# chaeyeongyun/VQ_SEG

Hardware: AMD Instinct MI355X
Metric: train images/sec @512x512 vqreptunet1x1 K=512 (higher is better)
Workload: dtype bf16; 1 GPU; CPS training iteration (2 x vqreptunet1x1, ResNet-50 encoder, K=[0,0,512,512,512], v1 recipe: 6 forwards + 4 backwards + 2 Adam steps) on 512x512x3 images -- BASELINE configs[2] (the metric's configuration): vqreptunet1x1 512x512, K = 512; labelled_per_gpu=32, unlabelled_per_gpu=32, parallelism=dp1, collectives=none (one process), conv_dtype=bf16

## Files before the change

### vq_seg_amd/csrc/conv_device.h

```cpp
#pragma once
#include <hip/hip_runtime.h>

#include "conv_kernels.h"

namespace vqseg {

typedef float f32x16 __attribute__((ext_vector_type(16)));
typedef float f32x4 __attribute__((ext_vector_type(4)));
typedef float f32x2 __attribute__((ext_vector_type(2)));
typedef __bf16 bf16x8 __attribute__((ext_vector_type(8)));
typedef __bf16 bf16x4 __attribute__((ext_vector_type(4)));
typedef unsigned int u32x4 __attribute__((ext_vector_type(4)));
typedef unsigned int u32x2 __attribute__((ext_vector_type(2)));

__device__ __forceinline__ unsigned int pack2(float a, float b) {
    const __bf16 x = (__bf16)a, y = (__bf16)b;
    return (unsigned int)__builtin_bit_cast(unsigned short, x) | ((unsigned int)__builtin_bit_cast(unsigned short, y) << 16);
}
__device__ __forceinline__ void unpack8(const u32x4 a, float (&v)[8]) {
#pragma unroll
    for (int e = 0; e < 4; ++e) {
        v[2 * e] = __builtin_bit_cast(float, a[e] << 16);
        v[2 * e + 1] = __builtin_bit_cast(float, a[e] & 0xFFFF0000u);
    }
// ... 9 lines not shown
__device__ __forceinline__ void split_row(long m, int hw, long M, int& n, int& rem) {
    if (M <= 0x7fffffffL) {
        const unsigned int um = (unsigned int)m;
        n = (int)(um / (unsigned int)hw);
        rem = (int)(um - (unsigned int)n * (unsigned int)hw);
    } else {
        n = (int)(m / hw);
        rem = (int)(m - (long)n * hw);
    }
}

__device__ __forceinline__ int reflect_idx(int i, int n) {
    if (i < 0) i = -i;
    if (i >= n) i = 2 * n - 2 - i;
    return i;
}

struct ASource {
    const char* src;
    int csrc, cbase;
};
__device__ __forceinline__ ASource a_source(const ConvArgs& p, int ci) {
    const bool second = ci >= p.C1;
    ASource a;
    a.src = reinterpret_cast<const char*>(second ? p.x2 : p.x);
    a.csrc = second ? (p.Cin - p.C1) : p.C1;
    a.cbase = second ? (ci - p.C1) : ci;
    if (p.s3_in) {
        const int cs2 = 2 * (second ? p.s3_cs2 : p.s3_cs1);
        a.csrc = cs2;
        if (a.cbase >= cs2) a.cbase -= cs2;
    }
    return a;
}

__device__ __forceinline__ long out_row(const ConvArgs& p, long m) {
    if (!p.omap) return m;
    const unsigned hw = (unsigned)(p.Ho * p.Wo), um = (unsigned)m;
    const unsigned n = um / hw, rem = um - n * hw;
    const unsigned oh = rem / (unsigned)p.Wo, ow = rem - oh * (unsigned)p.Wo;
    if (p.omap_fold) {
        const int i = 2 * (int)oh + p.omap_ph, j = 2 * (int)ow + p.omap_pw, H = p.omap_h, W = p.omap_w;
        const long body = (long)p.N * H * W;
        if (i >= 1 && j >= 1 && i <= H && j <= W) return ((long)n * H + i - 1) * W + j - 1;
        if (p.omap_fold == 1) {
            const int rl = W + 1 + H;
            if (i == 0 && j <= W) return body + (long)n * rl + j;
            if (j == 0 && i <= H) return body + (long)n * rl + W + i;
            return body + (long)p.N * rl;
        }
        return body;
    }
    return ((long)n * p.omap_h + 2 * oh + p.omap_ph) * p.omap_w + 2 * ow + p.omap_pw;
}

#ifndef GLDS_ABL
#define GLDS_ABL 0
#endif
struct LinearRows {
    long m0;
    __device__ __forceinline__ long operator()(int row) const { return m0 + row; }
};

template <int TBM, int BN, bool PRECISE, int MT, int NTT, int NT, int NTHR, typename RowMap = LinearRows, bool S3 = false, bool FAST = true>
__device__ __forceinline__ void conv_epilogue(f32x16 (&acc)[MT][NTT], const ConvArgs& p, char* smem, long M, long m0, int co0,
                                              int wm, int wn, int r, int h, int tid, RowMap row_to_m = LinearRows{-1}) {
// ... 256 lines not shown
```

### vq_seg_amd/csrc/conv_host.hip

```cpp
#include <hip/hip_runtime.h>
#include <stdlib.h>

#include "conv_internal.h"
#include "options.h"

namespace vqseg {

ConvOptions g_conv_opt;

static const Option CONV_OPTIONS[] = {
    {"conv3x3_patch_min_workgroups", &g_conv_opt.patch_min_wgs},
    {"conv_wgrad1x1_narrow", &g_conv_opt.wgrad1x1_narrow},
    {"stem_fused", &g_conv_opt.stem_fused, OPT_FLAG},
    {"conv_wgrad_round_pct", &g_conv_opt.wgrad_round_pct, OPT_RANGE_KEEP, 10, 400},
    {"conv_wgrad_xcd", &g_conv_opt.wgrad_xcd},
    {"conv_dgrad_s2_merge", &g_conv_opt.dgrad_s2_merge, OPT_FLAG},
    {"conv_wgrad3x3_fill", &g_conv_opt.wgrad3x3_fill},
    {"conv_wgrad3x3_stride2", &g_conv_opt.wgrad3x3_s2},
    {"conv_short_k_small_tile", &g_conv_opt.short_k_small},
    {"conv_short_k_single_buffer", &g_conv_opt.short_k_single},
    {"conv3x3_patch_unroll", &g_conv_opt.patch_unroll},
    {"conv_linear_prologue", &g_conv_opt.glds_lin, OPT_FLAG},
    {"conv_xcd_pair", &g_conv_opt.glds_pair},
    {"conv3x3_patch_xcd_pair", &g_conv_opt.patch_pair, OPT_FLAG},
    {"conv3x3_patch_chunk_stage", &g_conv_opt.patch_chunk_stage, OPT_FLAG},
    {"conv3x3_patch_tile512", &g_conv_opt.patch_tile512},
    {"conv3x3_patch_tile512_launches", &g_conv_opt.patch_tile512_launches},
    {"conv3x3_patch_tile512_min_workgroups", &g_conv_opt.patch_tile512_min_wgs},
    {"conv3x3_patch_wide_tile_s3", &g_conv_opt.patch_wide_s3, OPT_FLAG},
    {"conv3x3_patch_wide_tile", &g_conv_opt.patch_wide, OPT_FLAG},
    {"conv_last_variant", &g_conv_opt.last_variant},
};

int conv_set_option(const char* key, int value) { return apply_option(CONV_OPTIONS, key, value); }

struct ConvProfile {
    bool enabled = false;
    int capacity = 0, count = 0;
    hipEvent_t* ev = nullptr;
    double* flops = nullptr;
    int* kind = nullptr;
    int* shape = nullptr;
};
static ConvProfile g_cprof;

hipError_t conv_profile_begin(int capacity) {
    conv_profile_release();
    g_cprof.ev = (hipEvent_t*)malloc(sizeof(hipEvent_t) * 2 * (size_t)capacity);
    g_cprof.flops = (double*)malloc(sizeof(double) * (size_t)capacity);
    g_cprof.kind = (int*)malloc(sizeof(int) * (size_t)capacity);
    g_cprof.shape = (int*)malloc(sizeof(int) * 4 * (size_t)capacity);
    if (!g_cprof.ev || !g_cprof.flops || !g_cprof.kind || !g_cprof.shape) return hipErrorOutOfMemory;
    for (int i = 0; i < 2 * capacity; ++i) {
        hipError_t rc = hipEventCreate(&g_cprof.ev[i]);
        if (rc != hipSuccess) return rc;
    }
    g_cprof.capacity = capacity;
    g_cprof.count = 0;
    g_cprof.enabled = true;
    return hipSuccess;
}

void conv_profile_release() {
// ... 46 lines not shown
```

### vq_seg_amd/csrc/conv_igemm.hip

```cpp
#include <hip/hip_runtime.h>
#include <stdint.h>

#include "conv_device.h"
#include "conv_internal.h"

namespace vqseg {

constexpr int BM = 128;

template <int BN, bool PRECISE, int BK, bool S3 = false>
__global__ __launch_bounds__(256) void conv_igemm_kernel(const ConvArgs p) {
    constexpr int BKP = BK + 8;
    constexpr int NT = BN / 64;
    constexpr int WN = (BN >= 64) ? 2 : 1;
    constexpr int WM = 4 / WN;
    constexpr int MT = BM / (WM * 32);
    constexpr int NTT = (BN >= 64) ? NT : 1;
    constexpr int A_EPC = PRECISE ? 4 : 8;
    constexpr int A_CPR = BK / A_EPC;
    constexpr int A_RPP = 256 / A_CPR;
    constexpr int A_PASSES = BM / A_RPP;
    constexpr int B_CPR = BK / 8;
    constexpr int B_CHUNKS = BN * B_CPR * (PRECISE ? 2 : 1);
    constexpr int B_PER_THREAD = (B_CHUNKS + 255) / 256;
// ... 160 lines not shown
            }
#pragma unroll
            for (int a = 0; a < MT; ++a)
#pragma unroll
                for (int b = 0; b < NTT; ++b) {
                    if (PRECISE) {
                        acc[a][b] = __builtin_amdgcn_mfma_f32_32x32x16_bf16(a_lo[a], b_hi[b], acc[a][b], 0, 0, 0);
                        acc[a][b] = __builtin_amdgcn_mfma_f32_32x32x16_bf16(a_hi[a], b_lo[b], acc[a][b], 0, 0, 0);
                    }
                    acc[a][b] = __builtin_amdgcn_mfma_f32_32x32x16_bf16(a_hi[a], b_hi[b], acc[a][b], 0, 0, 0);
                }
        }
    };

    load_stage(0, a_r0, b_r0);
    if (n_stage > 1) load_stage(1, a_r1, b_r1);
    store_stage(0, a_r0, b_r0);
    __syncthreads();
    for (int s = 0; s < n_stage; s += 2) {
        if (s + 2 < n_stage) load_stage(s + 2, a_r0, b_r0);
        compute(0);
        if (s + 1 < n_stage) store_stage(1, a_r1, b_r1);
        __syncthreads();
        if (s + 1 >= n_stage) break;
        if (s + 3 < n_stage) load_stage(s + 3, a_r1, b_r1);
        compute(1);
        if (s + 2 < n_stage) store_stage(0, a_r0, b_r0);
        __syncthreads();
    }

    conv_epilogue<BM, BN, PRECISE, MT, NTT, NT, 256, LinearRows, S3, false>(acc, p, smem, M, m0, co0, wm, wn, r, h, tid);
}

template <int TBM, int BN, int NW, int NBUF, int MINW = 1, bool S3 = false, bool LIN = false, bool CLS = false>
__global__ __launch_bounds__(NW * 64, MINW) void conv_igemm_glds_kernel(const ConvArgs pk) {
    ConvArgs pc;
    long cls_tile0 = 0;
    if constexpr (CLS) {
        pc = pk;
        int c = 0;
        while (c + 1 < pk.n_cls && blockIdx.x >= pk.cls[c].tile_end) ++c;
        cls_tile0 = c ? pk.cls[c - 1].tile_end : 0;
        const ConvArgs::Cls& k = pk.cls[c];
        pc.KH = k.KH, pc.KW = k.KW, pc.pad = k.pad, pc.pad_w = k.pad_w, pc.Ho = k.Ho, pc.Wo = k.Wo;
        pc.omap_ph = k.ph, pc.omap_pw = k.pw;
        pc.w_hi = pk.w_hi + k.w_off;
    }
    const ConvArgs& p = CLS ? pc : pk;
    constexpr int BK = 64;
    constexpr int WN = (BN >= 256) ? 4 : (BN >= 64 ? 2 : 1);
    constexpr int WM = NW / WN;
    constexpr int MT = TBM / (WM * 32);
    constexpr int NT = (BN >= 64) ? BN / (WN * 32) : 1;
    constexpr int NTT = NT;
    constexpr int STAGE_BYTES = (TBM + BN) * BK * 2;
    constexpr int A_INSTR = TBM / 8 / NW;
    constexpr int B_ROWS_PER_WAVE = BN / NW;
    constexpr int B_INSTR = (B_ROWS_PER_WAVE + 7) / 8;

    extern __shared__ __attribute__((aligned(16))) char smem[];
    const int tid = threadIdx.x;
    const int lane = tid & 63;
    const int wave = __builtin_amdgcn_readfirstlane(tid >> 6);
    const int wm = wave / WN, wn = wave % WN;
    const int r = lane & 31, h = lane >> 5;

    const long M = (long)p.N * p.Ho * p.Wo;
    long m_tile = blockIdx.x - cls_tile0;
// ... 14 lines not shown
#pragma unroll
    for (int i = 0; i < A_INSTR; ++i) {
        const int trow = 8 * (A_INSTR * wave + i) + (lane >> 3);
        long m = m0 + trow;
        a_ok[i] = m < M;
        a_chunk[i] = slot ^ ((trow >> 1) & 7);
        if constexpr (LIN) {
            a_pix[i] = a_ok[i] ? m : -1;
            a_n[i] = a_oh[i] = a_ow[i] = 0;
        } else {
            if (!a_ok[i]) m = M - 1;
            int n, rem;
            split_row(m, p.Ho * p.Wo, M, n, rem);
            a_n[i] = n;
            a_oh[i] = rem / p.Wo;
            a_ow[i] = rem - a_oh[i] * p.Wo;
            if (p.ring) {
                const int q = rem, wp = p.ring_w, hp = p.ring_h;
                if (q < wp) a_oh[i] = 0, a_ow[i] = q;
                else if (q < 2 * wp) a_oh[i] = hp - 1, a_ow[i] = q - wp;
                else if (q < 2 * wp + hp - 2) a_oh[i] = 1 + (q - 2 * wp), a_ow[i] = 0;
                else a_oh[i] = 1 + (q - 2 * wp - (hp - 2)), a_ow[i] = wp - 1;
            }
        }
    }
    unsigned w_off[B_INSTR];
#pragma unroll
    for (int i = 0; i < B_INSTR; ++i) {
        const int b_row = B_ROWS_PER_WAVE * wave + 8 * i + (lane >> 3);
        const int co = co0 + b_row;
        const bool ok = co < p.Cout && b_row < B_ROWS_PER_WAVE * (wave + 1);
        w_off[i] = ok ? ((unsigned)co * (unsigned)(p.KH * p.KW * ((p.Cin + 31) / 32 * 32)) + (unsigned)((slot ^ ((b_row >> 1) & 7)) << 3)) * 2u
                      : ~0u;
    }

    f32x16 acc[MT][NTT];
#pragma unroll
    for (int a = 0; a < MT; ++a)
#pragma unroll
        for (int b = 0; b < NTT; ++b)
#pragma unroll
            for (int i = 0; i < 16; ++i) acc[a][b][i] = 0.0f;

    const int n_taps = p.KH * p.KW;
    const int cin_p = (p.Cin + 31) / 32 * 32;
    const int chunks_per_tap = p.Cin / BK;
    const int n_stage = n_taps * chunks_per_tap;
    const char* zero = reinterpret_cast<const char*>(g_zero_page);

    int cur_tap = LIN ? 0 : -1;
    auto set_tap = [&](int tap) {
        const int kh = tap / p.KW, kw = tap - kh * p.KW;
#pragma unroll
        for (int i = 0; i < A_INSTR; ++i) {
            int ih = a_oh[i] * p.stride - p.pad + kh;
            int iw = a_ow[i] * p.stride - p.pad_w + kw;
            bool ok = a_ok[i];
            if (p.reflect) {
                ih = reflect_idx(ih, p.H * p.up);
                iw = reflect_idx(iw, p.W * p.up);
            }
            if (p.up == 2) {
                ok = ok && ih >= 0 && iw >= 0 && !((ih | iw) & 1);
                ih >>= 1;
                iw >>= 1;
            }
            ok = ok && ih >= 0 && ih < p.H && iw >= 0 && iw < p.W;
            a_pix[i] = ok ? ((long)a_n[i] * p.H + ih) * p.W + iw : -1;
        }
        cur_tap = tap;
    };

    auto stage = [&](int s, int buf) {
        char* As = smem + buf * STAGE_BYTES;
        char* Bs = As + TBM * BK * 2;
        const int tap = s / chunks_per_tap;
        const int ci0 = (s - tap * chunks_per_tap) * BK;
        if (tap != cur_tap) set_tap(tap);
        const ASource as = a_source(p, ci0);
        const char* src = as.src;
        const int csrc = as.csrc, cbase = as.cbase;
#pragma unroll
        for (int i = 0; i < A_INSTR; ++i) {
            const long off = a_pix[i] * csrc + cbase + a_chunk[i] * 8;
            if (!(GLDS_ABL & 8)) glds16(a_pix[i] >= 0 ? src + off * 2 : zero, As + (A_INSTR * wave + i) * 1024);
        }
        const char* wbase = reinterpret_cast<const char*>(p.w_hi) + ((long)tap * cin_p + ci0) * 2;
#pragma unroll
        for (int i = 0; i < B_INSTR; ++i)
            glds16(w_off[i] != ~0u ? wbase + w_off[i] : zero, Bs + (B_ROWS_PER_WAVE * wave + 8 * i) * 128);
    };

    auto compute = [&](int buf) {
        const char* As = smem + buf * STAGE_BYTES;
        const char* Bs = As + TBM * BK * 2;
#pragma unroll MT * NTT >= 8 ? 1 : 4
        for (int kk = 0; kk < BK / 16; ++kk) {
            bf16x8 af[MT], bfr[NTT];
#pragma unroll
            for (int a = 0; a < MT; ++a) {
                const int row = (wm * MT + a) * 32 + r;
                const int sl = (kk * 2 + h) ^ ((row >> 1) & 7);
                af[a] = *reinterpret_cast<const bf16x8*>(As + row * 128 + sl * 16);
            }
#pragma unroll
            for (int b = 0; b < NTT; ++b) {
                const int row = (BN >= 64 ? (wn * NT + b) * 32 : 0) + r;
                const int sl = (kk * 2 + h) ^ ((row >> 1) & 7);
                bfr[b] = *reinterpret_cast<const bf16x8*>(Bs + row * 128 + sl * 16);
            }
#pragma unroll
            for (int a = 0; a < MT; ++a)
#pragma unroll
                for (int b = 0; b < NTT; ++b)
                    acc[a][b] = __builtin_amdgcn_mfma_f32_32x32x16_bf16(af[a], bfr[b], acc[a][b], 0, 0, 0);
        }
    };

    constexpr int G = A_INSTR + B_INSTR;
    auto wait_in_flight = [&](int stages) {
        if (stages >= 2 && NBUF >= 4) __builtin_amdgcn_s_waitcnt(((2 * G) & 0xF) | (((2 * G) >> 4) << 14) | 0x0F70);
        else if (stages >= 1 && NBUF >= 3) __builtin_amdgcn_s_waitcnt((G & 0xF) | ((G >> 4) << 14) | 0x0F70);
        else __builtin_amdgcn_s_waitcnt(0x0F70);
    };
    if constexpr (NBUF == 1) {
        for (int s = 0; s < n_stage; ++s) {
            stage(s, 0);
            __builtin_amdgcn_s_waitcnt(0x0F70);
// ... 114 lines not shown
    const __bf16* blrow = Bl + (wn * 32 + r) * KPW + h * 8;
#pragma unroll
    for (int kk = 0; kk < NK; ++kk) {
        const int g8 = 2 * kk + h;
        int kh = (g8 * 11) >> 5;
        const int j0 = 8 * (g8 - 3 * kh);
        if (kh > 6) kh = 6;
        const __bf16* src = strip + kh * ROW + j0;
        const bf16x8 b = *reinterpret_cast<const bf16x8*>(brow + kk * 16);
        bf16x8 bl;
        if constexpr (S3) bl = *reinterpret_cast<const bf16x8*>(blrow + kk * 16);
#pragma unroll
        for (int a = 0; a < 2; ++a) {
            const unsigned* sp = reinterpret_cast<const unsigned*>(src + 6 * ((wm * 2 + a) * 32 + r));
            const bf16x8 ah = __builtin_bit_cast(bf16x8, u32x4{sp[0], sp[1], sp[2], sp[3]});
            acc[a][0] = __builtin_amdgcn_mfma_f32_32x32x16_bf16(ah, b, acc[a][0], 0, 0, 0);
            if constexpr (S3) {
                const unsigned* sl = sp + PLANE / 2;
                const bf16x8 al = __builtin_bit_cast(bf16x8, u32x4{sl[0], sl[1], sl[2], sl[3]});
                acc[a][0] = __builtin_amdgcn_mfma_f32_32x32x16_bf16(al, b, acc[a][0], 0, 0, 0);
                acc[a][0] = __builtin_amdgcn_mfma_f32_32x32x16_bf16(ah, bl, acc[a][0], 0, 0, 0);
            }
        }
    }
    __syncthreads();
#if STEM_ABL & 2
    if (acc[0][0][0] != 12345.678f) return;
#endif
    conv_epilogue<TP, 64, false, 2, 1, 1, 256, LinearRows, S3, true>(acc, p, smem, M, m0, 0, wm, wn, r, h, tid);
}

template <int TBM, int BN, int NW, int NBUF, int MINW, bool LIN>
static void launch_glds_lin(const ConvArgs& a, hipStream_t st) {
    const int n_stage = a.KH * a.KW * (a.Cin / 64);
    size_t lds = (size_t)(TBM + BN) * 64 * 2 * (n_stage < NBUF ? n_stage : NBUF);
    const size_t out_tile = (size_t)TBM * (BN + 8) * 2 * (a.out_s3 ? 2 : 1);
    if (out_tile > lds) lds = out_tile;
    const long M = (long)a.N * a.Ho * a.Wo;
    const long m_tiles = (M + TBM - 1) / TBM;
    const int chunks = (a.Cout + BN - 1) / BN;
    if (chunks > 1 && chunks <= g_conv_opt.glds_pair && m_tiles < (1L << 30)) {
        ConvArgs b = a;
        b.pair_chunks = chunks;
        b.pair_tiles = (int)m_tiles;
        const dim3 grid1((unsigned)((m_tiles + 7) / 8 * 8 * chunks));
        g_conv_opt.last_variant = conv_variant_glds(TBM, BN, NW, NBUF, MINW, a.out_s3, LIN, false, true);
        if (a.out_s3) hipLaunchKernelGGL((conv_igemm_glds_kernel<TBM, BN, NW, NBUF, MINW, true, LIN>), grid1, dim3(NW * 64), lds, st, b);
        else hipLaunchKernelGGL((conv_igemm_glds_kernel<TBM, BN, NW, NBUF, MINW, false, LIN>), grid1, dim3(NW * 64), lds, st, b);
        return;
    }
    dim3 grid((unsigned)m_tiles, (unsigned)chunks);
    g_conv_opt.last_variant = conv_variant_glds(TBM, BN, NW, NBUF, MINW, a.out_s3, LIN, false, false);
    if (a.out_s3) hipLaunchKernelGGL((conv_igemm_glds_kernel<TBM, BN, NW, NBUF, MINW, true, LIN>), grid, dim3(NW * 64), lds, st, a);
    else hipLaunchKernelGGL((conv_igemm_glds_kernel<TBM, BN, NW, NBUF, MINW, false, LIN>), grid, dim3(NW * 64), lds, st, a);
}

template <int TBM, int BN, int NW, int NBUF, int MINW = 1>
static void launch_glds_t(const ConvArgs& a, hipStream_t st) {
    const bool lin = g_conv_opt.glds_lin && a.KH == 1 && a.KW == 1 && a.stride == 1 && a.pad == 0 && a.pad_w == 0 && a.up == 1 && !a.omap &&
                     a.Ho == a.H && a.Wo == a.W;
    if (lin) launch_glds_lin<TBM, BN, NW, NBUF, MINW, true>(a, st);
    else launch_glds_lin<TBM, BN, NW, NBUF, MINW, false>(a, st);
}

template <int BN, bool PRECISE, int BK>
static void launch_t(const ConvArgs& a, hipStream_t st) {
    constexpr int BKP = BK + 8;
    size_t lds = (size_t)(BM + BN) * BKP * 2 * (PRECISE ? 2 : 1) * 2;
    const size_t out_tile = (size_t)BM * (BN + (PRECISE ? 4 : 8)) * (PRECISE ? 4 : 2);
    if (out_tile > lds) lds = out_tile;
    const long M = (long)a.N * a.Ho * a.Wo;
    dim3 grid((unsigned)((M + BM - 1) / BM), (unsigned)((a.Cout + BN - 1) / BN));
    g_conv_opt.last_variant = conv_variant_igemm(BN, PRECISE, BK, !PRECISE && a.out_s3);
    if constexpr (!PRECISE) {
        if (a.out_s3) {
            const size_t s3_tile = (size_t)BM * (BN + 8) * 2 * 2;
            if (s3_tile > lds) lds = s3_tile;
            hipLaunchKernelGGL((conv_igemm_kernel<BN, PRECISE, BK, true>), grid, dim3(256), lds, st, a);
            return;
        }
    }
    hipLaunchKernelGGL((conv_igemm_kernel<BN, PRECISE, BK>), grid, dim3(256), lds, st, a);
}

#ifndef SHORTK_MINW
#define SHORTK_MINW 4
// ... 228 lines not shown
```

### vq_seg_amd/csrc/conv_internal.h

```cpp
#pragma once
#include "conv_kernels.h"

namespace vqseg {

struct ConvOptions {
    int glds_pair = 8;
    int glds_lin = 1;
    int patch_min_wgs = 128;
    int patch_pair = 0;
    int patch_chunk_stage = 1;
    int patch_wide_s3 = 1;
    int patch_wide = 1;
    int short_k_small = 1;
    int short_k_single = 8;
    int patch_tile512 = 2;
    int patch_tile512_min_wgs = 512;
    int patch_tile512_launches = 0;
    int patch_unroll = 1;
    int wgrad1x1_narrow = 1;
    int wgrad_round_pct = 100;
    int wgrad_xcd = 1;
    int wgrad3x3_fill = 1;
    int wgrad3x3_s2 = 1;
    int stem_fused = 1;
    int dgrad_s2_merge = 1;
    int last_variant = 0;
};
extern ConvOptions g_conv_opt;

enum ConvFamily { CONV_FAM_GLDS = 1, CONV_FAM_IGEMM = 2, CONV_FAM_PATCH = 3, CONV_FAM_WGRAD3X3 = 4, CONV_FAM_WGRAD1X1 = 5, CONV_FAM_WGRAD_TAP = 6 };
constexpr int conv_variant_id(int family, int d5, int d4, int d3, int d2, int d1, int flags) {
    return family << 24 | d5 << 20 | d4 << 16 | d3 << 12 | d2 << 8 | d1 << 4 | flags;
}
constexpr int conv_variant_glds(int tbm, int bn, int nw, int nbuf, int minw, bool s3, bool lin, bool cls, bool pair) {
    return conv_variant_id(CONV_FAM_GLDS, tbm / 128, bn / 32, nw, nbuf, minw, s3 * 8 + lin * 4 + cls * 2 + pair);
}
constexpr int conv_variant_igemm(int bn, bool precise, int bk, bool s3) { return conv_variant_id(CONV_FAM_IGEMM, 0, bn / 32, 0, bk / 32, precise, s3 * 8); }
constexpr int conv_variant_patch(int bn, int nbw, bool unroll, int ck, bool s3, int tbm, bool pair) {
    return conv_variant_id(CONV_FAM_PATCH, tbm / 256, bn / 32, nbw, ck / 32, unroll, s3 * 8 + pair);
}
constexpr int conv_variant_wgrad3x3(int cot, int cit, int stride, bool xcd) { return conv_variant_id(CONV_FAM_WGRAD3X3, 0, cot, cit, stride, 0, xcd); }
constexpr int conv_variant_wgrad1x1(int cot, int cit, bool xcd) { return conv_variant_id(CONV_FAM_WGRAD1X1, 0, cot, cit, 0, 0, xcd); }
constexpr int conv_variant_wgrad_tap(int tm, int tn, bool precise) { return conv_variant_id(CONV_FAM_WGRAD_TAP, 0, tm, tn, 0, precise, 0); }

class ConvProfileScope {
public:
    ConvProfileScope(hipStream_t st, double flops, int kind, int shape0, int shape1, int shape2, int shape3);
    ~ConvProfileScope();
    ConvProfileScope(const ConvProfileScope&) = delete;
    ConvProfileScope& operator=(const ConvProfileScope&) = delete;

private:
    hipStream_t st_;
    int slot_;
};

bool launch_conv3x3_patch(const ConvArgs& a, bool k64, hipStream_t st);

}
```

### vq_seg_amd/csrc/conv_patch.hip

```cpp
#include <hip/hip_runtime.h>
#include <stdint.h>

#include "conv_device.h"
#include "conv_internal.h"

namespace vqseg {

#ifndef PATCH_ABL
#define PATCH_ABL 0
#endif
#ifndef CONV_SETPRIO
#define CONV_SETPRIO 0
#endif

template <int BN, int NBW, bool UNROLL_TAPS, int CK = 64, bool S3 = false, int TBM = 256>
__global__ __launch_bounds__(512) void conv3x3_patch_kernel(const ConvArgs p) {
    constexpr int NW = 8;
    static_assert(TBM == 256 || (TBM == 512 && CK == 32), "512-pixel tiles stage 32-channel chunks (two patch buffers must fit the LDS)");
    constexpr int PATCH_PX = TBM == 256 ? 344 : 616;
    constexpr int NT = BN >= 128 ? 2 : 1;
    constexpr int WN = BN / (32 * NT), WM = NW / WN;
    constexpr int MT = TBM / (WM * 32);
    constexpr int ROWB = CK * 2;
    constexpr int RPI = 1024 / ROWB;
    constexpr int KS = CK / 16;
    constexpr int PI = (PATCH_PX + RPI * NW - 1) / (RPI * NW);
    constexpr int PATCH_BYTES = PI * NW * 1024;
    constexpr int W_ROWS = (BN * ROWB >= NW * 1024) ? BN : NW * 1024 / ROWB;
    constexpr int W_BYTES = W_ROWS * ROWB;
    constexpr int WI = W_BYTES / 1024 / NW;
    static_assert(W_BYTES % (1024 * NW) == 0 && (CK == 64 || CK == 32), "weight tile must split evenly over the waves");
    constexpr bool CHUNK_STAGE = NBW == 0;
    constexpr int WT_BYTES = CHUNK_STAGE ? BN * ROWB : W_BYTES;
    constexpr int WCI = 9 * BN * ROWB / 1024, WCW = (WCI + NW - 1) / NW;
    static_assert(!CHUNK_STAGE || (BN * ROWB) % 1024 == 0, "a tap's weight tile must be whole DMA instructions");
    auto swz = [](int row) { return CK == 64 ? ((row >> 1) & 7) : ((row >> 2) & 3); };

    extern __shared__ __attribute__((aligned(16))) char smem[];
    char* const patch0 = smem;
    char* const wring = smem + ((CHUNK_STAGE && p.Cin / CK == 1) ? 1 : 2) * PATCH_BYTES;
    const int tid = threadIdx.x, lane = tid & 63;
    const int wave = __builtin_amdgcn_readfirstlane(tid >> 6);
    const int wm = wave / WN, wn = wave % WN;
    const int r = lane & 31, h = lane >> 5;

    const int tw_shift = (p.W & 31) == 0 ? 5 : 4;
    const int TW = 1 << tw_shift, TH = TBM >> tw_shift, PW = TW + 2, PH = TH + 2;
    const int tiles_x = p.W >> tw_shift, tiles_y = p.H / TH;
    int tile_id = blockIdx.x, co_chunk = blockIdx.y;
    if (p.pair_chunks > 0) {
        const unsigned group = 8u * (unsigned)p.pair_chunks, within = blockIdx.x % group;
        tile_id = (int)(blockIdx.x / group) * 8 + (int)(within & 7u);
        co_chunk = (int)(within >> 3);
        if (tile_id >= p.pair_tiles) return;
    }
    int t = tile_id;
    const int txi = t % tiles_x;
    t /= tiles_x;
    const int tyi = t % tiles_y;
    const int n = t / tiles_y;
    const int oh0 = tyi * TH, ow0 = txi * TW;
    const int co0 = co_chunk * BN;

    const int slot = lane & (ROWB / 16 - 1), lrow = lane / (ROWB / 16);
    unsigned w_off[WI];
#pragma unroll
    for (int i = 0; i < WI; ++i) {
        const int row = RPI * (wave * WI + i) + lrow;
        int co = co0 + row;
        co = co < p.Cout ? co : p.Cout - 1;
        w_off[i] = ((unsigned)co * (unsigned)(9 * ((p.Cin + 31) / 32 * 32)) + (unsigned)((slot ^ swz(row)) << 3)) * 2u;
    }
    int a_pp[MT];
#pragma unroll
    for (int a = 0; a < MT; ++a) {
        const int row = (wm * MT + a) * 32 + r;
        a_pp[a] = (row >> tw_shift) * PW + (row & (TW - 1));
    }

    f32x16 acc[MT][NT];
#pragma unroll
    for (int a = 0; a < MT; ++a)
#pragma unroll
        for (int b = 0; b < NT; ++b)
#pragma unroll
            for (int i = 0; i < 16; ++i) acc[a][b][i] = 0.0f;

    const int cin_p = (p.Cin + 31) / 32 * 32;
    const int n_chunks = p.Cin / CK;
    const int n_stage = n_chunks * 9;
    const char* zero = reinterpret_cast<const char*>(g_zero_page);

    auto issue_patch = [&](int chunk, int i) {
        const int pp = RPI * (wave + NW * i) + lrow;
        const int pr = pp / PW, pc = pp - pr * PW;
        int ih = oh0 - 1 + pr, iw = ow0 - 1 + pc;
        bool ok = pr < PH;
        if (p.reflect && ok) {
            ih = reflect_idx(ih, p.H);
            iw = reflect_idx(iw, p.W);
        }
        ok = ok && ih >= 0 && ih < p.H && iw >= 0 && iw < p.W;
        const long pix = ((long)n * p.H + ih) * p.W + iw;
        const int ci0 = chunk * CK;
        const ASource as = a_source(p, ci0);
        const char* src = as.src;
        const int csrc = as.csrc, cbase = as.cbase;
        const long off = pix * csrc + cbase + ((slot ^ swz(pp)) << 3);
        glds16(ok ? src + off * 2 : zero, patch0 + (chunk & 1) * PATCH_BYTES + (wave + NW * i) * 1024);
    };
    auto issue_weights = [&](int chunk, int tap, int wslot) {
        char* Bs = wring + wslot * W_BYTES;
        const char* sbase = reinterpret_cast<const char*>(p.w_hi) + ((long)tap * cin_p + chunk * CK) * 2;
#pragma unroll
        for (int i = 0; i < WI; ++i) glds16(sbase + w_off[i], Bs + (wave * WI + i) * 1024);
    };
    auto compute = [&](int chunk, int tapoff, const char* Bs) {
        const char* Ps = patch0 + (chunk & 1) * PATCH_BYTES;
#pragma unroll
        for (int kk = 0; kk < KS; ++kk) {
            bf16x8 af[MT], bfr[NT];
#pragma unroll
            for (int a = 0; a < MT; ++a) {
                const int pp = a_pp[a] + tapoff;
                af[a] = *reinterpret_cast<const bf16x8*>(Ps + pp * ROWB + (((kk * 2 + h) ^ swz(pp)) << 4));
            }
#pragma unroll
            for (int b = 0; b < NT; ++b) {
                const int row = (wn * NT + b) * 32 + r;
                bfr[b] = *reinterpret_cast<const bf16x8*>(Bs + row * ROWB + (((kk * 2 + h) ^ swz(row)) << 4));
            }
#if CONV_SETPRIO
            __builtin_amdgcn_s_setprio(1);
#endif
#pragma unroll
            for (int a = 0; a < MT; ++a)
#pragma unroll
                for (int b = 0; b < NT; ++b)
                    acc[a][b] = __builtin_amdgcn_mfma_f32_32x32x16_bf16(af[a], bfr[b], acc[a][b], 0, 0, 0);
#if CONV_SETPRIO
            __builtin_amdgcn_s_setprio(0);
#endif
        }
    };

    if constexpr (CHUNK_STAGE) {
        auto issue_chunk = [&](int chunk) {
#pragma unroll
            for (int i = 0; i < PI; ++i) issue_patch(chunk, i);
            char* wb = wring + (chunk & 1) * (9 * WT_BYTES);
#pragma unroll
            for (int i = 0; i < WCW; ++i) {
                const int j = wave * WCW + i;
                if (j < WCI) {
                    const int tap = j / (BN * ROWB / 1024), rg = j % (BN * ROWB / 1024);
                    const int row = RPI * rg + lrow;
                    int co = co0 + row;
                    co = co < p.Cout ? co : p.Cout - 1;
                    const unsigned short* wp = p.w_hi + (long)co * (9L * cin_p) + (long)tap * cin_p + chunk * CK + ((slot ^ swz(row)) << 3);
                    glds16(reinterpret_cast<const char*>(wp), wb + j * 1024);
                }
            }
        };
        issue_chunk(0);
        for (int chunk = 0; chunk < n_chunks; ++chunk) {
            __builtin_amdgcn_s_waitcnt(0x0F70);
            stage_barrier();
            if (chunk + 1 < n_chunks) issue_chunk(chunk + 1);
            const char* wb = wring + (chunk & 1) * (9 * WT_BYTES);
#pragma unroll
            for (int tap = 0; tap < 9; ++tap) compute(chunk, (tap / 3) * PW + tap % 3, wb + tap * WT_BYTES);
        }
        __syncthreads();
        const long M = (long)p.N * p.H * p.W;
        const TileRows rows{((long)n * p.H + oh0) * p.W + ow0, tw_shift, p.W};
        conv_epilogue<TBM, BN, false, MT, NT, NT, NW * 64, TileRows, S3>(acc, p, smem, M, (long)tile_id * TBM, co0, wm, wn, r, h, tid, rows);
        return;
    }
#pragma unroll
    for (int i = 0; i < PI; ++i) issue_patch(0, i);
#pragma unroll
    for (int s = 0; s < NBW - 1; ++s)
        if (s < n_stage) issue_weights(s / 9, s % 9, s);

    int wslot = 0;
    for (int chunk = 0; chunk < n_chunks; ++chunk) {
        const bool more = chunk + 1 < n_chunks;
#pragma unroll UNROLL_TAPS ? 9 : 1
        for (int tap = 0; tap < 9; ++tap) {
            const int s = chunk * 9 + tap;
            int young = 0;
#pragma unroll
// ... 19 lines not shown
                    const int c2 = tap + NBW - 1 >= 9 ? chunk + 1 : chunk, t2 = tap + NBW - 1 >= 9 ? tap + NBW - 1 - 9 : tap + NBW - 1;
                    int ws2 = wslot + NBW - 1;
                    if (ws2 >= NBW) ws2 -= NBW;
                    issue_weights(c2, t2, ws2);
                }
            };
            if (NBW < 4) issue_next();
            compute(chunk, (tap / 3) * PW + tap % 3, wring + wslot * W_BYTES);
            if (NBW >= 4) issue_next();
            wslot = wslot == NBW - 1 ? 0 : wslot + 1;
        }
    }
    __syncthreads();
    const long M = (long)p.N * p.H * p.W;
    const TileRows rows{((long)n * p.H + oh0) * p.W + ow0, tw_shift, p.W};
    conv_epilogue<TBM, BN, false, MT, NT, NT, NW * 64, TileRows, S3>(acc, p, smem, M, (long)tile_id * TBM, co0, wm, wn, r, h, tid, rows);
}

static bool conv3x3_patch_ok(const ConvArgs& a) {
    if (a.omap || a.pad_w != a.pad) return false;
    if (a.KH != 3 || a.KW != 3 || a.stride != 1 || a.pad != 1 || a.up != 1 || a.Ho != a.H || a.Wo != a.W) return false;
    const int ck = a.Cin % 64 == 0 && (a.C1 == a.Cin || a.C1 % 64 == 0) ? 64 : 32;
    if (a.Cin % ck || (a.C1 != a.Cin && a.C1 % ck) || (a.Cout % 128 && a.Cout != 64 && a.Cout != 32)) return false;
    const int tw = (a.W % 32 == 0) ? 32 : 16, th = 256 / tw;
    if (a.W % tw || a.H % th) return false;
    const int bn = a.Cout % 128 == 0 ? 128 : a.Cout;
    return (long)a.N * (a.H / th) * (a.W / tw) * (a.Cout / bn) >= g_conv_opt.patch_min_wgs;
}

template <int BN, int NBW, bool UNROLL_TAPS, int CK = 64, int TBM = 256>
static void launch_patch_t(const ConvArgs& a, hipStream_t st) {
    constexpr int ROWB = CK * 2, RPI = 1024 / ROWB, PI = ((TBM == 256 ? 344 : 616) + RPI * 8 - 1) / (RPI * 8);
    constexpr int W_ROWS = (BN * ROWB >= 8 * 1024) ? BN : 8 * 1024 / ROWB;
    size_t lds = 2 * (size_t)PI * 8 * 1024 + (size_t)NBW * W_ROWS * ROWB;
    if (NBW == 0) {
        const int nb = a.Cin / CK > 1 ? 2 : 1;
        lds = (size_t)nb * ((size_t)PI * 8 * 1024 + 9 * (size_t)BN * ROWB);
    }
    size_t out_tile = (size_t)TBM * (BN + 8) * 2 * (a.out_s3 ? 2 : 1);
    if (a.out_s3 && out_tile > 160u * 1024u) out_tile = (size_t)TBM * (BN / 2 + 8) * 4;
    if (out_tile > lds) lds = out_tile;
    const int tw = (a.W % 32 == 0) ? 32 : 16, th = TBM / tw;
    const long tiles = (long)a.N * (a.H / th) * (a.W / tw);
    const int chunks = a.Cout / BN;
    if (g_conv_opt.patch_pair && chunks > 1) {
        ConvArgs b = a;
        b.pair_chunks = chunks;
        b.pair_tiles = (int)tiles;
        const dim3 grid1((unsigned)((tiles + 7) / 8 * 8 * chunks));
        g_conv_opt.last_variant = conv_variant_patch(BN, NBW, UNROLL_TAPS, CK, a.out_s3, TBM, true);
        if (a.out_s3) hipLaunchKernelGGL((conv3x3_patch_kernel<BN, NBW, UNROLL_TAPS, CK, true, TBM>), grid1, dim3(512), lds, st, b);
        else hipLaunchKernelGGL((conv3x3_patch_kernel<BN, NBW, UNROLL_TAPS, CK, false, TBM>), grid1, dim3(512), lds, st, b);
        return;
    }
    dim3 grid((unsigned)tiles, (unsigned)chunks);
    g_conv_opt.last_variant = conv_variant_patch(BN, NBW, UNROLL_TAPS, CK, a.out_s3, TBM, false);
    if (a.out_s3) hipLaunchKernelGGL((conv3x3_patch_kernel<BN, NBW, UNROLL_TAPS, CK, true, TBM>), grid, dim3(512), lds, st, a);
    else hipLaunchKernelGGL((conv3x3_patch_kernel<BN, NBW, UNROLL_TAPS, CK, false, TBM>), grid, dim3(512), lds, st, a);
}

static bool conv3x3_tile512_ok(const ConvArgs& a, int bn) {
    if (a.Cin % 32 || (a.C1 != a.Cin && a.C1 % 32)) return false;
    const int tw = (a.W % 32 == 0) ? 32 : 16, th = 512 / tw;
    if (a.W % tw || a.H % th) return false;
    if (a.out_s3 && (size_t)512 * (bn + 8) * 2 * 2 > 160 * 1024) return false;
    return (long)a.N * (a.H / th) * (a.W / tw) * (a.Cout / bn) >= g_conv_opt.patch_tile512_min_wgs;
}

bool launch_conv3x3_patch(const ConvArgs& a, bool k64, hipStream_t st) {
    if (!conv3x3_patch_ok(a)) return false;
    if ((g_conv_opt.patch_tile512 & 2) && (a.Cout == 32 || (a.Cout == 64 && a.Cin >= 64)) && conv3x3_tile512_ok(a, a.Cout)) {
        ++g_conv_opt.patch_tile512_launches;
        if (a.Cout == 64) launch_patch_t<64, 0, true, 32, 512>(a, st);
        else launch_patch_t<32, 0, true, 32, 512>(a, st);
    } else if (!k64) {
        if (g_conv_opt.patch_chunk_stage && a.Cout == 64) launch_patch_t<64, 0, true, 32>(a, st);
        else if (g_conv_opt.patch_chunk_stage && a.Cout == 32) launch_patch_t<32, 0, true, 32>(a, st);
        else if (g_conv_opt.patch_chunk_stage && a.Cin == 32) launch_patch_t<128, 0, true, 32>(a, st);
        else if (a.Cout == 64) launch_patch_t<64, 3, true, 32>(a, st);
        else if (a.Cout == 32) launch_patch_t<32, 3, true, 32>(a, st);
        else launch_patch_t<128, 3, true, 32>(a, st);
    } else {
        const int tw = (a.W % 32 == 0) ? 32 : 16, th = 256 / tw;
        const long tiles = (long)a.N * (a.H / th) * (a.W / tw);
        if (a.Cout == 64) launch_patch_t<64, 3, true>(a, st);
        else if (a.Cout == 32) launch_patch_t<32, 3, true>(a, st);
        else if (a.Cout % 256 == 0 && g_conv_opt.patch_wide && (!a.out_s3 || g_conv_opt.patch_wide_s3) && tiles * (a.Cout / 256) >= g_conv_opt.patch_min_wgs)
            launch_patch_t<256, 2, false>(a, st);
        else if (g_conv_opt.patch_unroll == 2)
            launch_patch_t<128, 4, true>(a, st);
// ... 10 lines not shown
```

Baseline: 445.9 images/sec.

## Stage split-3 hi/lo channel halves together and issue three MFMAs per chunk

For split-3 (bf16 hi/lo) inputs and outputs, the patch and glds conv kernels now load matching hi and lo channel halves of a chunk into one LDS stage. Each k-step then issues the lo*hi, hi*lo and hi*hi MFMAs from that single stage, instead of running over the doubled channel dimension as separate chunks. The intent is to cut LDS staging traffic and the number of pipeline stages for split-3 precise convolutions. In exchange it adds address arithmetic with a flag bit packed into the weight offsets, and adds extra template instantiations. It is enabled by default for CK=64 patch kernels and for glds kernels with TBM<256.

Result: no change. 449.1 images/sec, median of 6 (+0.7%).

```diff
diff --git a/vq_seg_amd/csrc/conv_device.h b/vq_seg_amd/csrc/conv_device.h
--- a/vq_seg_amd/csrc/conv_device.h
+++ b/vq_seg_amd/csrc/conv_device.h
@@ -65,6 +65,19 @@
         if (a.cbase >= cs2) a.cbase -= cs2;
     }
     return a;
+}
+
+struct S3Chunk {
+    bool second;
+    int cs, c, wbase;
+};
+__device__ __forceinline__ S3Chunk s3_chunk(const ConvArgs& p, int c0) {
+    S3Chunk s;
+    s.second = c0 >= p.s3_cs1;
+    s.cs = s.second ? p.s3_cs2 : p.s3_cs1;
+    s.c = s.second ? c0 - p.s3_cs1 : c0;
+    s.wbase = s.second ? 3 * p.s3_cs1 : 0;
+    return s;
 }
 
 __device__ __forceinline__ long out_row(const ConvArgs& p, long m) {
diff --git a/vq_seg_amd/csrc/conv_host.hip b/vq_seg_amd/csrc/conv_host.hip
--- a/vq_seg_amd/csrc/conv_host.hip
+++ b/vq_seg_amd/csrc/conv_host.hip
@@ -29,6 +29,7 @@
     {"conv3x3_patch_tile512_min_workgroups", &g_conv_opt.patch_tile512_min_wgs},
     {"conv3x3_patch_wide_tile_s3", &g_conv_opt.patch_wide_s3, OPT_FLAG},
     {"conv3x3_patch_wide_tile", &g_conv_opt.patch_wide, OPT_FLAG},
+    {"conv_s3_fused", &g_conv_opt.s3_fused, OPT_RANGE_FAIL, 0, 15},
     {"conv_last_variant", &g_conv_opt.last_variant},
 };
 
diff --git a/vq_seg_amd/csrc/conv_igemm.hip b/vq_seg_amd/csrc/conv_igemm.hip
--- a/vq_seg_amd/csrc/conv_igemm.hip
+++ b/vq_seg_amd/csrc/conv_igemm.hip
@@ -216,8 +216,9 @@
     conv_epilogue<BM, BN, PRECISE, MT, NTT, NT, 256, LinearRows, S3, false>(acc, p, smem, M, m0, co0, wm, wn, r, h, tid);
 }
 
-template <int TBM, int BN, int NW, int NBUF, int MINW = 1, bool S3 = false, bool LIN = false, bool CLS = false>
+template <int TBM, int BN, int NW, int NBUF, int MINW = 1, bool S3 = false, bool LIN = false, bool CLS = false, bool FUSE3 = false>
 __global__ __launch_bounds__(NW * 64, MINW) void conv_igemm_glds_kernel(const ConvArgs pk) {
+    static_assert(!FUSE3 || (S3 && !CLS), "fused split-3 chunks: split-3 input and output");
     ConvArgs pc;
     long cls_tile0 = 0;
     if constexpr (CLS) {
@@ -298,6 +299,10 @@
         const bool ok = co < p.Cout && b_row < B_ROWS_PER_WAVE * (wave + 1);
         w_off[i] = ok ? ((unsigned)co * (unsigned)(p.KH * p.KW * ((p.Cin + 31) / 32 * 32)) + (unsigned)((slot ^ ((b_row >> 1) & 7)) << 3)) * 2u
                       : ~0u;
+        if constexpr (FUSE3) {
+            const int ls = slot ^ ((b_row >> 1) & 7);
+            if (ok) w_off[i] = (((unsigned)co * (unsigned)(p.KH * p.KW * ((p.Cin + 31) / 32 * 32)) + (unsigned)((ls & 3) << 3)) * 2u) | (ls >= 4 ? 1u : 0u);
+        }
     }
 
     f32x16 acc[MT][NTT];
@@ -310,7 +315,7 @@
 
     const int n_taps = p.KH * p.KW;
     const int cin_p = (p.Cin + 31) / 32 * 32;
-    const int chunks_per_tap = p.Cin / BK;
+    const int chunks_per_tap = FUSE3 ? (p.s3_cs1 + p.s3_cs2) / (BK / 2) : p.Cin / BK;
     const int n_stage = n_taps * chunks_per_tap;
     const char* zero = reinterpret_cast<const char*>(g_zero_page);
 
@@ -343,6 +348,21 @@
         const int tap = s / chunks_per_tap;
         const int ci0 = (s - tap * chunks_per_tap) * BK;
         if (tap != cur_tap) set_tap(tap);
+        if constexpr (FUSE3) {
+            const S3Chunk sc = s3_chunk(p, (s - tap * chunks_per_tap) * (BK / 2));
+            const char* src = reinterpret_cast<const char*>(sc.second ? p.x2 : p.x);
+#pragma unroll
+            for (int i = 0; i < A_INSTR; ++i) {
+                const long off = a_pix[i] * (2 * sc.cs) + sc.c + (a_chunk[i] >= 4 ? sc.cs : 0) + (a_chunk[i] & 3) * 8;
+                glds16(a_pix[i] >= 0 ? src + off * 2 : zero, As + (A_INSTR * wave + i) * 1024);
+            }
+            const char* wbase = reinterpret_cast<const char*>(p.w_hi) + ((long)tap * cin_p + sc.wbase + sc.c) * 2;
+            const unsigned lo_bytes = 4u * (unsigned)sc.cs;
+#pragma unroll
+            for (int i = 0; i < B_INSTR; ++i)
+                glds16(w_off[i] != ~0u ? wbase + ((w_off[i] & ~1u) + ((w_off[i] & 1u) ? lo_bytes : 0u)) : zero, Bs + (B_ROWS_PER_WAVE * wave + 8 * i) * 128);
+            return;
+        }
         const ASource as = a_source(p, ci0);
         const char* src = as.src;
         const int csrc = as.csrc, cbase = as.cbase;
@@ -360,6 +380,37 @@
     auto compute = [&](int buf) {
         const char* As = smem + buf * STAGE_BYTES;
         const char* Bs = As + TBM * BK * 2;
+        if constexpr (FUSE3) {
+#pragma unroll MT * NTT >= 8 ? 1 : 2
+            for (int kk = 0; kk < BK / 32; ++kk) {
+                bf16x8 ah[MT], al[MT], bh[NTT], bl[NTT];
+#pragma unroll
+                for (int a = 0; a < MT; ++a) {
+                    const int row = (wm * MT + a) * 32 + r;
+                    ah[a] = *reinterpret_cast<const bf16x8*>(As + row * 128 + (((kk * 2 + h) ^ ((row >> 1) & 7)) << 4));
+                    al[a] = *reinterpret_cast<const bf16x8*>(As + row * 128 + (((4 + kk * 2 + h) ^ ((row >> 1) & 7)) << 4));
+                }
+#pragma unroll
+                for (int b = 0; b < NTT; ++b) {
+                    const int row = (BN >= 64 ? (wn * NT + b) * 32 : 0) + r;
+                    bh[b] = *reinterpret_cast<const bf16x8*>(Bs + row * 128 + (((kk * 2 + h) ^ ((row >> 1) & 7)) << 4));
+                    bl[b] = *reinterpret_cast<const bf16x8*>(Bs + row * 128 + (((4 + kk * 2 + h) ^ ((row >> 1) & 7)) << 4));
+                }
+#pragma unroll
+                for (int a = 0; a < MT; ++a)
+#pragma unroll
+                    for (int b = 0; b < NTT; ++b) acc[a][b] = __builtin_amdgcn_mfma_f32_32x32x16_bf16(al[a], bh[b], acc[a][b], 0, 0, 0);
+#pragma unroll
+                for (int a = 0; a < MT; ++a)
+#pragma unroll
+                    for (int b = 0; b < NTT; ++b) acc[a][b] = __builtin_amdgcn_mfma_f32_32x32x16_bf16(ah[a], bl[b], acc[a][b], 0, 0, 0);
+#pragma unroll
+                for (int a = 0; a < MT; ++a)
+#pragma unroll
+                    for (int b = 0; b < NTT; ++b) acc[a][b] = __builtin_amdgcn_mfma_f32_32x32x16_bf16(ah[a], bh[b], acc[a][b], 0, 0, 0);
+            }
+            return;
+        }
 #pragma unroll MT * NTT >= 8 ? 1 : 4
         for (int kk = 0; kk < BK / 16; ++kk) {
             bf16x8 af[MT], bfr[NTT];
@@ -540,7 +591,8 @@
 
 template <int TBM, int BN, int NW, int NBUF, int MINW, bool LIN>
 static void launch_glds_lin(const ConvArgs& a, hipStream_t st) {
-    const int n_stage = a.KH * a.KW * (a.Cin / 64);
+    const bool fused = (g_conv_opt.s3_fused & 2) && (TBM < 256 || (g_conv_opt.s3_fused & 8)) && a.s3_in && a.out_s3 && !a.ring && a.s3_cs1 % 32 == 0 && a.s3_cs2 % 32 == 0;
+    const int n_stage = a.KH * a.KW * (fused ? (a.s3_cs1 + a.s3_cs2) / 32 : a.Cin / 64);
     size_t lds = (size_t)(TBM + BN) * 64 * 2 * (n_stage < NBUF ? n_stage : NBUF);
     const size_t out_tile = (size_t)TBM * (BN + 8) * 2 * (a.out_s3 ? 2 : 1);
     if (out_tile > lds) lds = out_tile;
@@ -552,14 +604,16 @@
         b.pair_chunks = chunks;
         b.pair_tiles = (int)m_tiles;
         const dim3 grid1((unsigned)((m_tiles + 7) / 8 * 8 * chunks));
-        g_conv_opt.last_variant = conv_variant_glds(TBM, BN, NW, NBUF, MINW, a.out_s3, LIN, false, true);
-        if (a.out_s3) hipLaunchKernelGGL((conv_igemm_glds_kernel<TBM, BN, NW, NBUF, MINW, true, LIN>), grid1, dim3(NW * 64), lds, st, b);
+        g_conv_opt.last_variant = conv_variant_glds(TBM, BN, NW, NBUF, MINW, a.out_s3, LIN, false, true, fused);
+        if (fused) hipLaunchKernelGGL((conv_igemm_glds_kernel<TBM, BN, NW, NBUF, MINW, true, LIN, false, true>), grid1, dim3(NW * 64), lds, st, b);
+        else if (a.out_s3) hipLaunchKernelGGL((conv_igemm_glds_kernel<TBM, BN, NW, NBUF, MINW, true, LIN>), grid1, dim3(NW * 64), lds, st, b);
         else hipLaunchKernelGGL((conv_igemm_glds_kernel<TBM, BN, NW, NBUF, MINW, false, LIN>), grid1, dim3(NW * 64), lds, st, b);
         return;
     }
     dim3 grid((unsigned)m_tiles, (unsigned)chunks);
-    g_conv_opt.last_variant = conv_variant_glds(TBM, BN, NW, NBUF, MINW, a.out_s3, LIN, false, false);
-    if (a.out_s3) hipLaunchKernelGGL((conv_igemm_glds_kernel<TBM, BN, NW, NBUF, MINW, true, LIN>), grid, dim3(NW * 64), lds, st, a);
+    g_conv_opt.last_variant = conv_variant_glds(TBM, BN, NW, NBUF, MINW, a.out_s3, LIN, false, false, fused);
+    if (fused) hipLaunchKernelGGL((conv_igemm_glds_kernel<TBM, BN, NW, NBUF, MINW, true, LIN, false, true>), grid, dim3(NW * 64), lds, st, a);
+    else if (a.out_s3) hipLaunchKernelGGL((conv_igemm_glds_kernel<TBM, BN, NW, NBUF, MINW, true, LIN>), grid, dim3(NW * 64), lds, st, a);
     else hipLaunchKernelGGL((conv_igemm_glds_kernel<TBM, BN, NW, NBUF, MINW, false, LIN>), grid, dim3(NW * 64), lds, st, a);
 }
 
diff --git a/vq_seg_amd/csrc/conv_internal.h b/vq_seg_amd/csrc/conv_internal.h
--- a/vq_seg_amd/csrc/conv_internal.h
+++ b/vq_seg_amd/csrc/conv_internal.h
@@ -24,6 +24,7 @@
     int wgrad3x3_s2 = 1;
     int stem_fused = 1;
     int dgrad_s2_merge = 1;
+    int s3_fused = 3;
     int last_variant = 0;
 };
 extern ConvOptions g_conv_opt;
@@ -32,12 +33,12 @@
 constexpr int conv_variant_id(int family, int d5, int d4, int d3, int d2, int d1, int flags) {
     return family << 24 | d5 << 20 | d4 << 16 | d3 << 12 | d2 << 8 | d1 << 4 | flags;
 }
-constexpr int conv_variant_glds(int tbm, int bn, int nw, int nbuf, int minw, bool s3, bool lin, bool cls, bool pair) {
-    return conv_variant_id(CONV_FAM_GLDS, tbm / 128, bn / 32, nw, nbuf, minw, s3 * 8 + lin * 4 + cls * 2 + pair);
+constexpr int conv_variant_glds(int tbm, int bn, int nw, int nbuf, int minw, bool s3, bool lin, bool cls, bool pair, bool fuse3 = false) {
+    return conv_variant_id(CONV_FAM_GLDS, tbm / 128, bn / 32, nw, nbuf, minw + fuse3 * 8, s3 * 8 + lin * 4 + cls * 2 + pair);
 }
 constexpr int conv_variant_igemm(int bn, bool precise, int bk, bool s3) { return conv_variant_id(CONV_FAM_IGEMM, 0, bn / 32, 0, bk / 32, precise, s3 * 8); }
-constexpr int conv_variant_patch(int bn, int nbw, bool unroll, int ck, bool s3, int tbm, bool pair) {
-    return conv_variant_id(CONV_FAM_PATCH, tbm / 256, bn / 32, nbw, ck / 32, unroll, s3 * 8 + pair);
+constexpr int conv_variant_patch(int bn, int nbw, bool unroll, int ck, bool s3, int tbm, bool pair, bool fuse3 = false) {
+    return conv_variant_id(CONV_FAM_PATCH, tbm / 256, bn / 32, nbw, ck / 32, unroll, s3 * 8 + fuse3 * 4 + pair);
 }
 constexpr int conv_variant_wgrad3x3(int cot, int cit, int stride, bool xcd) { return conv_variant_id(CONV_FAM_WGRAD3X3, 0, cot, cit, stride, 0, xcd); }
 constexpr int conv_variant_wgrad1x1(int cot, int cit, bool xcd) { return conv_variant_id(CONV_FAM_WGRAD1X1, 0, cot, cit, 0, 0, xcd); }
diff --git a/vq_seg_amd/csrc/conv_patch.hip b/vq_seg_amd/csrc/conv_patch.hip
--- a/vq_seg_amd/csrc/conv_patch.hip
+++ b/vq_seg_amd/csrc/conv_patch.hip
@@ -13,9 +13,10 @@
 #define CONV_SETPRIO 0
 #endif
 
-template <int BN, int NBW, bool UNROLL_TAPS, int CK = 64, bool S3 = false, int TBM = 256>
+template <int BN, int NBW, bool UNROLL_TAPS, int CK = 64, bool S3 = false, int TBM = 256, bool FUSE3 = false>
 __global__ __launch_bounds__(512) void conv3x3_patch_kernel(const ConvArgs p) {
     constexpr int NW = 8;
+    static_assert(!FUSE3 || S3, "fused split-3 chunks: split-3 input and output");
     static_assert(TBM == 256 || (TBM == 512 && CK == 32), "512-pixel tiles stage 32-channel chunks (two patch buffers must fit the LDS)");
     constexpr int PATCH_PX = TBM == 256 ? 344 : 616;
     constexpr int NT = BN >= 128 ? 2 : 1;
@@ -23,7 +24,9 @@
     constexpr int MT = TBM / (WM * 32);
     constexpr int ROWB = CK * 2;
     constexpr int RPI = 1024 / ROWB;
-    constexpr int KS = CK / 16;
+    constexpr int KS = FUSE3 ? CK / 32 : CK / 16;
+    constexpr int CL = FUSE3 ? CK / 2 : CK;
+    constexpr int HS = ROWB / 32;
     constexpr int PI = (PATCH_PX + RPI * NW - 1) / (RPI * NW);
     constexpr int PATCH_BYTES = PI * NW * 1024;
     constexpr int W_ROWS = (BN * ROWB >= NW * 1024) ? BN : NW * 1024 / ROWB;
@@ -38,7 +41,7 @@
 
     extern __shared__ __attribute__((aligned(16))) char smem[];
     char* const patch0 = smem;
-    char* const wring = smem + ((CHUNK_STAGE && p.Cin / CK == 1) ? 1 : 2) * PATCH_BYTES;
+    char* const wring = smem + ((CHUNK_STAGE && (FUSE3 ? (p.s3_cs1 + p.s3_cs2) / CL : p.Cin / CK) == 1) ? 1 : 2) * PATCH_BYTES;
     const int tid = threadIdx.x, lane = tid & 63;
     const int wave = __builtin_amdgcn_readfirstlane(tid >> 6);
     const int wm = wave / WN, wn = wave % WN;
@@ -69,7 +72,9 @@
         const int row = RPI * (wave * WI + i) + lrow;
         int co = co0 + row;
         co = co < p.Cout ? co : p.Cout - 1;
-        w_off[i] = ((unsigned)co * (unsigned)(9 * ((p.Cin + 31) / 32 * 32)) + (unsigned)((slot ^ swz(row)) << 3)) * 2u;
+        const int ls = slot ^ swz(row);
+        if constexpr (FUSE3) w_off[i] = (((unsigned)co * (unsigned)(9 * ((p.Cin + 31) / 32 * 32)) + (unsigned)((ls & (HS - 1)) << 3)) * 2u) | (ls >= HS ? 1u : 0u);
+        else w_off[i] = ((unsigned)co * (unsigned)(9 * ((p.Cin + 31) / 32 * 32)) + (unsigned)(ls << 3)) * 2u;
     }
     int a_pp[MT];
 #pragma unroll
@@ -87,7 +92,7 @@
             for (int i = 0; i < 16; ++i) acc[a][b][i] = 0.0f;
 
     const int cin_p = (p.Cin + 31) / 32 * 32;
-    const int n_chunks = p.Cin / CK;
+    const int n_chunks = FUSE3 ? (p.s3_cs1 + p.s3_cs2) / CL : p.Cin / CK;
     const int n_stage = n_chunks * 9;
     const char* zero = reinterpret_cast<const char*>(g_zero_page);
 
@@ -102,21 +107,67 @@
         }
         ok = ok && ih >= 0 && ih < p.H && iw >= 0 && iw < p.W;
         const long pix = ((long)n * p.H + ih) * p.W + iw;
-        const int ci0 = chunk * CK;
-        const ASource as = a_source(p, ci0);
-        const char* src = as.src;
-        const int csrc = as.csrc, cbase = as.cbase;
-        const long off = pix * csrc + cbase + ((slot ^ swz(pp)) << 3);
+        const char* src;
+        long off;
+        if constexpr (FUSE3) {
+            const S3Chunk sc = s3_chunk(p, chunk * CL);
+            const int ls = slot ^ swz(pp);
+            src = reinterpret_cast<const char*>(sc.second ? p.x2 : p.x);
+            off = pix * (2 * sc.cs) + sc.c + (ls >= HS ? sc.cs : 0) + ((ls & (HS - 1)) << 3);
+        } else {
+            const ASource as = a_source(p, chunk * CK);
+            src = as.src;
+            off = pix * as.csrc + as.cbase + ((slot ^ swz(pp)) << 3);
+        }
         glds16(ok ? src + off * 2 : zero, patch0 + (chunk & 1) * PATCH_BYTES + (wave + NW * i) * 1024);
     };
     auto issue_weights = [&](int chunk, int tap, int wslot) {
         char* Bs = wring + wslot * W_BYTES;
-        const char* sbase = reinterpret_cast<const char*>(p.w_hi) + ((long)tap * cin_p + chunk * CK) * 2;
-#pragma unroll
-        for (int i = 0; i < WI; ++i) glds16(sbase + w_off[i], Bs + (wave * WI + i) * 1024);
+        if constexpr (FUSE3) {
+            const S3Chunk sc = s3_chunk(p, chunk * CL);
+            const char* sbase = reinterpret_cast<const char*>(p.w_hi) + ((long)tap * cin_p + sc.wbase + sc.c) * 2;
+            const unsigned lo_bytes = 4u * (unsigned)sc.cs;
+#pragma unroll
+            for (int i = 0; i < WI; ++i) glds16(sbase + ((w_off[i] & ~1u) + ((w_off[i] & 1u) ? lo_bytes : 0u)), Bs + (wave * WI + i) * 1024);
+        } else {
+            const char* sbase = reinterpret_cast<const char*>(p.w_hi) + ((long)tap * cin_p + chunk * CK) * 2;
+#pragma unroll
+            for (int i = 0; i < WI; ++i) glds16(sbase + w_off[i], Bs + (wave * WI + i) * 1024);
+        }
     };
     auto compute = [&](int chunk, int tapoff, const char* Bs) {
         const char* Ps = patch0 + (chunk & 1) * PATCH_BYTES;
+        if constexpr (FUSE3) {
+#pragma unroll
+            for (int kk = 0; kk < KS; ++kk) {
+                bf16x8 ah[MT], al[MT], bh[NT], bl[NT];
+#pragma unroll
+                for (int a = 0; a < MT; ++a) {
+                    const int pp = a_pp[a] + tapoff;
+                    ah[a] = *reinterpret_cast<const bf16x8*>(Ps + pp * ROWB + (((kk * 2 + h) ^ swz(pp)) << 4));
+                    al[a] = *reinterpret_cast<const bf16x8*>(Ps + pp * ROWB + (((HS + kk * 2 + h) ^ swz(pp)) << 4));
+                }
+#pragma unroll
+                for (int b = 0; b < NT; ++b) {
+                    const int row = (wn * NT + b) * 32 + r;
+                    bh[b] = *reinterpret_cast<const bf16x8*>(Bs + row * ROWB + (((kk * 2 + h) ^ swz(row)) << 4));
+                    bl[b] = *reinterpret_cast<const bf16x8*>(Bs + row * ROWB + (((HS + kk * 2 + h) ^ swz(row)) << 4));
+                }
+#pragma unroll
+                for (int a = 0; a < MT; ++a)
+#pragma unroll
+                    for (int b = 0; b < NT; ++b) acc[a][b] = __builtin_amdgcn_mfma_f32_32x32x16_bf16(al[a], bh[b], acc[a][b], 0, 0, 0);
+#pragma unroll
+                for (int a = 0; a < MT; ++a)
+#pragma unroll
+                    for (int b = 0; b < NT; ++b) acc[a][b] = __builtin_amdgcn_mfma_f32_32x32x16_bf16(ah[a], bl[b], acc[a][b], 0, 0, 0);
+#pragma unroll
+                for (int a = 0; a < MT; ++a)
+#pragma unroll
+                    for (int b = 0; b < NT; ++b) acc[a][b] = __builtin_amdgcn_mfma_f32_32x32x16_bf16(ah[a], bh[b], acc[a][b], 0, 0, 0);
+            }
+            return;
+        }
 #pragma unroll
         for (int kk = 0; kk < KS; ++kk) {
             bf16x8 af[MT], bfr[NT];
@@ -158,6 +209,11 @@
                     int co = co0 + row;
                     co = co < p.Cout ? co : p.Cout - 1;
                     const unsigned short* wp = p.w_hi + (long)co * (9L * cin_p) + (long)tap * cin_p + chunk * CK + ((slot ^ swz(row)) << 3);
+                    if constexpr (FUSE3) {
+                        const S3Chunk sc = s3_chunk(p, chunk * CL);
+                        const int ls = slot ^ swz(row);
+                        wp = p.w_hi + (long)co * (9L * cin_p) + (long)tap * cin_p + sc.wbase + sc.c + (ls >= HS ? 2 * sc.cs : 0) + ((ls & (HS - 1)) << 3);
+                    }
                     glds16(reinterpret_cast<const char*>(wp), wb + j * 1024);
                 }
             }
@@ -243,9 +299,11 @@
 static void launch_patch_t(const ConvArgs& a, hipStream_t st) {
     constexpr int ROWB = CK * 2, RPI = 1024 / ROWB, PI = ((TBM == 256 ? 344 : 616) + RPI * 8 - 1) / (RPI * 8);
     constexpr int W_ROWS = (BN * ROWB >= 8 * 1024) ? BN : 8 * 1024 / ROWB;
+    const bool fused = (g_conv_opt.s3_fused & 1) && (CK == 64 || (g_conv_opt.s3_fused & 4)) && a.s3_in && a.out_s3 && a.s3_cs1 % (CK / 2) == 0 && a.s3_cs2 % (CK / 2) == 0;
+    const int n_chunks = fused ? (a.s3_cs1 + a.s3_cs2) / (CK / 2) : a.Cin / CK;
     size_t lds = 2 * (size_t)PI * 8 * 1024 + (size_t)NBW * W_ROWS * ROWB;
     if (NBW == 0) {
-        const int nb = a.Cin / CK > 1 ? 2 : 1;
+        const int nb = n_chunks > 1 ? 2 : 1;
         lds = (size_t)nb * ((size_t)PI * 8 * 1024 + 9 * (size_t)BN * ROWB);
     }
     size_t out_tile = (size_t)TBM * (BN + 8) * 2 * (a.out_s3 ? 2 : 1);
@@ -259,14 +317,16 @@
         b.pair_chunks = chunks;
         b.pair_tiles = (int)tiles;
         const dim3 grid1((unsigned)((tiles + 7) / 8 * 8 * chunks));
-        g_conv_opt.last_variant = conv_variant_patch(BN, NBW, UNROLL_TAPS, CK, a.out_s3, TBM, true);
-        if (a.out_s3) hipLaunchKernelGGL((conv3x3_patch_kernel<BN, NBW, UNROLL_TAPS, CK, true, TBM>), grid1, dim3(512), lds, st, b);
+        g_conv_opt.last_variant = conv_variant_patch(BN, NBW, UNROLL_TAPS, CK, a.out_s3, TBM, true, fused);
+        if (fused) hipLaunchKernelGGL((conv3x3_patch_kernel<BN, NBW, UNROLL_TAPS, CK, true, TBM, true>), grid1, dim3(512), lds, st, b);
+        else if (a.out_s3) hipLaunchKernelGGL((conv3x3_patch_kernel<BN, NBW, UNROLL_TAPS, CK, true, TBM>), grid1, dim3(512), lds, st, b);
         else hipLaunchKernelGGL((conv3x3_patch_kernel<BN, NBW, UNROLL_TAPS, CK, false, TBM>), grid1, dim3(512), lds, st, b);
         return;
     }
     dim3 grid((unsigned)tiles, (unsigned)chunks);
-    g_conv_opt.last_variant = conv_variant_patch(BN, NBW, UNROLL_TAPS, CK, a.out_s3, TBM, false);
-    if (a.out_s3) hipLaunchKernelGGL((conv3x3_patch_kernel<BN, NBW, UNROLL_TAPS, CK, true, TBM>), grid, dim3(512), lds, st, a);
+    g_conv_opt.last_variant = conv_variant_patch(BN, NBW, UNROLL_TAPS, CK, a.out_s3, TBM, false, fused);
+    if (fused) hipLaunchKernelGGL((conv3x3_patch_kernel<BN, NBW, UNROLL_TAPS, CK, true, TBM, true>), grid, dim3(512), lds, st, a);
+    else if (a.out_s3) hipLaunchKernelGGL((conv3x3_patch_kernel<BN, NBW, UNROLL_TAPS, CK, true, TBM>), grid, dim3(512), lds, st, a);
     else hipLaunchKernelGGL((conv3x3_patch_kernel<BN, NBW, UNROLL_TAPS, CK, false, TBM>), grid, dim3(512), lds, st, a);
 }
 
```
